# castacks/mvs_gi

Measured on AMD Instinct MI355X. Metric: stereo frames/sec/GPU (G16V, 3-cam, D=16) + inv-dist L1 vs reference, higher is better.
Workload: dtype f16x3 (split-fp16 MFMA operands: 11 + 11 significant bits, f32 accumulate/activations)

## Files before the change

### mvs_gi_amd/csrc/conv3d.hip

```cpp
#include "common.hpp"
#include "conv_common.hpp"
#include "conv3d_variants.hpp"
#ifdef MVSGI_STAMPS
#include <cstdio>
#include <cstdlib>
#endif

namespace {

__global__ void pack_head_weights_kernel(const float* __restrict__ w, float* __restrict__ wp, int Cin) {
    const int idx = blockIdx.x * 256 + threadIdx.x;
    if (idx >= 27 * Cin) return;
    const int tap = idx / Cin, ci = idx % Cin;
    wp[idx] = w[ci * 27 + tap];
}

#include "conv3d_f32mfma.hpp"
#include "conv3d_bf16x3.hpp"


__global__ __launch_bounds__(256) void conv3d_head_kernel(ConvArgs a, int dchunk, int nd) {
    constexpr int TH = 8, TW = 32, ITH = TH + 2, ITW = TW + 2, PV = ITH * ITW;
    constexpr int NT = (PV + 31) / 32;
    constexpr int TPW = (NT + 3) / 4;
// ... 199 lines not shown
    MVSGI_REQUIRE((long long)a.Hin * a.Win * a.Cin < (1ll << 31), "conv3d(head): plane too large for 32-bit offsets");
    hipLaunchKernelGGL(conv3d_head_kernel, dim3((unsigned)nt), dim3(256), lds_bytes, st, a, dchunk, (int)nd);
    return mvsgi::check_launch("mvsgi_conv3d_f32(head)");
}

int launch_direct(const ConvArgs& a, hipStream_t st) {
    const long long vox = (long long)a.B * a.Do * a.Ho * a.Wo;
    if (a.Cout == 1) {
        hipLaunchKernelGGL((conv3d_direct_kernel<1>), dim3((unsigned)mvsgi::cdiv(vox, 256)), dim3(256), 0, st, a);
    } else {
        const long long total = vox * mvsgi::cdiv(a.Cout, 4);
        hipLaunchKernelGGL((conv3d_direct_kernel<4>), dim3((unsigned)mvsgi::cdiv(total, 256)), dim3(256), 0, st, a);
    }
    return mvsgi::check_launch("mvsgi_conv3d_f32(direct)");
}

bool v32_applies(const ConvArgs& a) {
    if (a.Cout % 32 || a.Cin % 16 || a.stride != 1) return false;
    const long long big = (long long)a.B * mvsgi::cdiv(a.Do, 4) * mvsgi::cdiv(a.Ho, 4) * mvsgi::cdiv(a.Wo, 16);
    const long long mid = (long long)a.B * mvsgi::cdiv(a.Do, 2) * mvsgi::cdiv(a.Ho, 4) * mvsgi::cdiv(a.Wo, 16);
    return a.Cout == 32 ? big >= 384 : mid * mvsgi::cdiv(a.Cout, 64) >= 384;
}

int select_variant_up2(const ConvArgs& a, int w_layout) {
    if (w_layout == MVSGI_CONV_BF16X3_D32) {
        const int base = a.Cin % 32 ? V_COUNT : select_variant_up2(a, MVSGI_CONV_BF16X3);
        const bool d2 = a.Do == 2;
        if (base == B3U_N64) return d2 ? B3DU2_N64 : B3DU_N64;
        if (base == B3U_N96) return d2 ? B3DU2_N96 : B3DU_N96;
        mvsgi::fail("mvsgi_conv3d_up2_f32: the 32-channel-slice kernels do not apply to this problem (see mvsgi_conv3d_up2_d32_applies)");
        return V_COUNT;
    }
    const bool c16_layout = w_layout == MVSGI_CONV_BF16X3_C16;
    if (w_layout == MVSGI_CONV_BF16X3_V32) {
        if (!v32_applies(a) || !a.wp) { mvsgi::fail("mvsgi_conv3d_up2_f32: the 32x32x16 kernel does not apply to this problem"); return V_COUNT; }
        return a.Cout == 32 ? B3VU_N32 : B3VU_N64;
    }
    if (a.Cin % 16 || a.Cout % 16) {
        mvsgi::fail("mvsgi_conv3d_up2_f32: Cin, Cout must be multiples of 16 (got %d, %d)", a.Cin, a.Cout);
        return V_COUNT;
    }
    if (!a.wp) { mvsgi::fail("mvsgi_conv3d_up2_f32: needs w_packed (bf16x3 layout)"); return V_COUNT; }
    const int CT = a.Cout / 16;
    const long long big = (long long)a.B * mvsgi::cdiv(a.Do, 4) * mvsgi::cdiv(a.Ho, 4) * mvsgi::cdiv(a.Wo, 16);
    const long long mid = (long long)a.B * mvsgi::cdiv(a.Do, 2) * mvsgi::cdiv(a.Ho, 4) * mvsgi::cdiv(a.Wo, 16);
    if (CT == 1) return c16_layout ? B3PU_N16 : B3U_N16;
    if (CT == 2) {
        if (big >= 384) return B3U_N32;
        const long long cus = mvsgi::device_cus(), r32 = mvsgi::cdiv(big, cus), rm = mvsgi::cdiv(mid, cus);
        return 157 * (100 + 85 * (r32 - 1)) < 100 * (100 + 85 * (rm - 1)) ? B3U_N32 : B3U_N32_M;
    }
    if (CT == 3) return B3U_N48;
    if (CT % 6 == 0 && mid * (CT / 6) >= 384) return B3U_N96;
    if (CT % 2 == 0 && (long long)a.B * mvsgi::cdiv(a.Do, 2) * mvsgi::cdiv(a.Ho, 2) * mvsgi::cdiv(a.Wo, 16) * (CT / 2) <= mvsgi::device_cus())
        return B3U_N32_TB;
    return B3U_N64;
}

int select_variant(const ConvArgs& a, int impl);

int d32_variant(const ConvArgs& a) {
    if (a.stride != 1 || a.Cin % 32 || a.Cout % 16) return V_COUNT;
    ConvArgs b = a;
    static const float dummy = 0.f;
    if (!b.wp) b.wp = reinterpret_cast<const f32x4*>(&dummy);
    const bool d2 = a.Do == 2;
    switch (select_variant(b, MVSGI_CONV_BF16X3)) {
        case B3_N64: return d2 ? B3D2_N64 : B3D_N64;
        case B3_N64_H5: return d2 ? B3D2_N64_H5 : B3D_N64_H5;
        case B3_N64_W8: return d2 ? B3D2_N64_W8 : B3D_N64_W8;
        case B3_N96: return d2 ? B3D2_N96 : B3D_N96;
        case B3_N96_H5: return d2 ? B3D2_N96_H5 : B3D_N96_H5;
        case B3_N96_W8: return d2 ? B3D2_N96_W8 : B3D_N96_W8;
        case B3_N128_P: return B3D_N128_P;
        case B3_N128_PH5: return B3D_N128_PH5;
        case B3_N128_PW8: return B3D_N128_PW8;
        case B3_N192_PH5: return B3D_N192_PH5;
        case B3_N192_PW8: return B3D_N192_PW8;
        case B3_N16_TW: return d2 && a.Cout % 32 == 0 ? B3D2_N32_TB : V_COUNT;
        case B3_N32_TB: return d2 ? B3D2_N32_TB : B3D_N32_TB;
        case B3_N64_S: return d2 ? B3D2_N64_S : B3D_N64_S;
        default: return V_COUNT;
    }
}

// ... 398 lines not shown
```

### mvs_gi_amd/csrc/conv3d_bf16x3.hpp

```cpp
#pragma once
#ifndef MVSGI_ABL
#define MVSGI_ABL 0
#endif

#include "split_fmt.hpp"

constexpr int kVSB = 80;

__device__ __forceinline__ void split_bf16x4(const f32x4 x, u32x2& hi, u32x2& lo) {
#pragma unroll
    for (int p = 0; p < 2; ++p) {
        const f32x2 v = {x[2 * p], x[2 * p + 1]};
        const unsigned hb = __builtin_bit_cast(unsigned, __builtin_convertvector(v, bf16x2));
        const f32x2 hf = {__builtin_bit_cast(float, hb << 16), __builtin_bit_cast(float, hb & 0xffff0000u)};
        hi[p] = hb;
        float r0 = v[0] - hf[0], r1 = v[1] - hf[1];
        asm volatile("" : "+v"(r0));
        asm volatile("" : "+v"(r1));
        lo[p] = __builtin_bit_cast(unsigned, __builtin_convertvector(f32x2{r0, r1}, bf16x2));
    }
}
__device__ __forceinline__ f32x4 fma4(const f32x4 a, const f32x4 b, const f32x4 c) {
    f32x4 r;
#pragma unroll
// ... 142 lines not shown
    if (idx >= total) return;
    const int lane = (int)(idx & 63);
    long long r = idx >> 6;
    const int tap = (int)(r % 27);
    r /= 27;
    const int ct = (int)(r % CT);
    const int cc = (int)(r / CT);
    const int co = ct * 32 + (lane & 31);
    const int ci = cc * 16 + (lane >> 5) * 8;
    u16x8 hi, lo;
    for (int j = 0; j < 8; ++j) {
        const float v = w[((long long)co * Cin + ci + j) * 27 + tap];
        unsigned short h_, l_;
        split_weight(v, f16, h_, l_);
        hi[j] = h_;
        lo[j] = l_;
    }
    const long long o = ((((long long)cc * CT + ct) * 27 + tap) * 2) * 64 + lane;
    wp[o] = __builtin_bit_cast(bf16x8, hi);
    wp[o + 64] = __builtin_bit_cast(bf16x8, lo);
}

template <int NW, int MW, int WM, int WN, int TD, int TH, int TW, int S, int KD, bool UPS, bool PLANE, bool V32, bool WLDS, bool F16, bool D32 = false, int DK = 3, int BRD = 0>
__device__ __forceinline__ void conv3d_x3_body(const ConvArgs& a) {
    static_assert(!WLDS || (WN == 1 && KD == 3 && !UPS && !PLANE && !V32 && S == 1 && NW == 1 && MW <= 2), "LDS-staged weights: one shared cout tile, one or two voxel tiles per wave");
    static_assert(!V32 || (S == 1 && KD == 3 && TW == 16 && TH % 2 == 0 && !PLANE), "32x32x16 schedule: stride 1, 16-wide even bricks");
    static_assert(!PLANE || (NW == 1 && WN == 1 && WM == 4 && TH == 4 && MW == TD && TW == 16 && S == 1 && KD == 3),
                  "plane schedule: Cout == 16, 4 h-rows x TD planes x 16 w per brick");
    static_assert(!UPS || (S == 1 && KD == 3 && TD % 2 == 0 && TH % 2 == 0 && TW % 2 == 0),
                  "fused upsample: stride 1, even bricks (halo bricks are whole 2x2x2 cells)");
    static_assert(WM * WN == 4, "4 consumer waves per workgroup");
    static_assert(WM * MW * (V32 ? 32 : 16) == TD * TH * TW, "brick must be covered by the voxel tiles");
    static_assert(KD == 3 || (KD == 1 && TD == 1), "2-D bricks are one plane thick");
    constexpr int SD = KD == 1 ? 1 : S;
    static_assert(!D32 || (KD == 3 && S == 1 && !PLANE && !V32 && !WLDS), "32-channel slices: stride-1 3x3x3 variants (plain or fused upsample) only");
    static_assert(DK == 3 || (D32 && DK >= 1 && (TD == 1 ? DK <= 2 : (TD == 2 && WM == 2 && MW * 16 == TH * TW))), "depth skip: one- or two-plane bricks whose waves own whole planes");
    constexpr bool DKU = D32 && TD == 1 && DK == 2;
    constexpr int kTaps = KD * 9, kPairs = D32 ? 9 * DK : pairs_of(KD);
    constexpr int kWBlk = D32 ? 27 : kPairs;
    constexpr int ITD = (TD - 1) * SD + KD, ITH = (TH - 1) * S + 3, ITW = (TW - 1) * S + 3;
    constexpr int IV = ITD * ITH * ITW;
    constexpr int QB = D32 ? 3 : 2;
    constexpr int NIT = (IV * (1 << QB) + 255) / 256;
    constexpr int ROWP = V32 ? ((ITW * kVSB + 255) / 256) * 256 : ITW * kVSB;
    constexpr int SUB = ITD * ITH * ROWP;
    constexpr int BUF = D32 ? 2 * SUB : SUB;
    constexpr int WB = WLDS ? (MW * NW == 1 ? 8 : 4) :
// ... 2 lines not shown
                       NW <= 2 ? 4 : 2;
    constexpr int LA = WB - 1;
    constexpr int NSLOT = ((kPairs + WB - 1) / WB) * WB;
    static_assert(NSLOT % WB == 0 && NSLOT >= kPairs, "pipeline geometry");
    constexpr bool RPRE = MW * NW <= 8;
#ifndef MVSGI_WARM
#define MVSGI_WARM 0
#endif
    constexpr bool WARM = MVSGI_WARM && KD == 3 && !UPS && !PLANE && !V32 && !WLDS && S == 1 && MW * NW <= 2;

    constexpr int WBYTES = WLDS ? NW * kPairs * 2048 : 0;
    constexpr int BUFW = BUF + WBYTES;
    constexpr int WARM_LDS = 2 * BUFW;
    extern __shared__ __attribute__((aligned(16))) unsigned char ldsb[];
    float satm = 0.f;

    const int tid = threadIdx.x, lane = tid & 63;
    const int wave = __builtin_amdgcn_readfirstlane(tid >> 6);
    const bool producer = wave >= 4;
    const int CT = a.Cout / (V32 ? 32 : 16);
    const int ny = (CT + WN * NW - 1) / (WN * NW);
    const int nchunks = a.Cin / (D32 ? 32 : 16);
    const int total = a.total_units;
    const int G = gridDim.x;
    const int nmine = (total - (int)blockIdx.x + G - 1) / G;
    const int U = nmine * nchunks;
#ifdef MVSGI_STAMPS
    int nst = 0;
#define STAMP()                                                                                     \
    if (a.dbg && blockIdx.x == 8 && nst < 120) {                                                    \
        unsigned long long t_;                                                                      \
        asm volatile("s_memtime %0\n\ts_waitcnt lgkmcnt(0)" : "=s"(t_)::"memory");                  \
        if (lane == 0) a.dbg[wave * 128 + nst] = t_;                                                \
        nst++;                                                                                      \
    }
#else
#define STAMP()
#endif
    STAMP()

#define MVSGI_DECODE_DH(T, OD, OH, B) { OD = (T % a.tiles_d) * TD + a.od_off; T /= a.tiles_d; OH = (T % a.tiles_h) * TH; B = T / a.tiles_h; }
#define MVSGI_DECODE(ID, CB, B, OD, OH, OW)                       \
    {                                                             \
        int t_ = xcd_remap((ID), total);                          \
        CB = t_ % ny;                                             \
        t_ /= ny;                                                 \
        OW = (t_ % a.tiles_w) * TW;                               \
        t_ /= a.tiles_w;                                          \
// ... 18 lines not shown
            f32x4 crA[NITU][8], crB[NITU][8];
            unsigned imA[NITU], imB[NITU];
#define MVSGI_PLAN_UPS(UNIT)                                                                            \
            {                                                                                           \
                int cb_, b_, od_, oh_, ow_;                                                             \
                MVSGI_DECODE(UNIT, cb_, b_, od_, oh_, ow_)                                              \
                (void)cb_;                                                                              \
                _Pragma("unroll") for (int it = 0; it < NITU; ++it) {                                   \
                    const int c = MVSGI_UPS_CQ(it) >> QB;                                               \
                    const int cw = c % CW, ch = (c / CW) % CH, cd = c / (CW * CH);                      \
                    const int gd = od_ - 1 + 2 * cd, gh = oh_ - 1 + 2 * ch, gw = ow_ - 1 + 2 * cw;      \
                    lo_d[it] = (gd - 1) >> 1;                                                           \
                    lo_h[it] = (gh - 1) >> 1;                                                           \
                    lo_w[it] = (gw - 1) >> 1;                                                           \
                    inmask[it] = (gd >= 0 && gd < a.Din ? 1u : 0u) | (gd + 1 < a.Din ? 2u : 0u) |       \
                                 (gh >= 0 && gh < a.Hin ? 4u : 0u) | (gh + 1 < a.Hin ? 8u : 0u) |       \
                                 (gw >= 0 && gw < a.Win ? 16u : 0u) | (gw + 1 < a.Win ? 32u : 0u);      \
                }                                                                                       \
                xb = a.x + (long long)b_ * Dl * Hl * Wl * a.Cin;                                        \
            }
#define MVSGI_CLAMP(V, N) ((V) < 0 ? 0 : ((V) > (N) - 1 ? (N) - 1 : (V)))
            int k2 = 0, cc2 = 0;
#define MVSGI_ISSUE_UPS_BEGIN()                                                                         \
            if (cc2 == 0 && k2 > 0) { MVSGI_PLAN_UPS((int)blockIdx.x + k2 * G) }
#define MVSGI_ISSUE_UPS1(CR, IM, IT)                                                                    \
            {                                                                                           \
                const int q = MVSGI_UPS_CQ(IT) & ((1 << QB) - 1);                                       \
                const bool live = MVSGI_UPS_LIVE(IT);                                                   \
                const int d0 = live ? MVSGI_CLAMP(lo_d[IT], Dl) : 0, d1 = live ? MVSGI_CLAMP(lo_d[IT] + 1, Dl) : 0; \
                const int h0 = live ? MVSGI_CLAMP(lo_h[IT], Hl) : 0, h1 = live ? MVSGI_CLAMP(lo_h[IT] + 1, Hl) : 0; \
                const int w0 = live ? MVSGI_CLAMP(lo_w[IT], Wl) : 0, w1 = live ? MVSGI_CLAMP(lo_w[IT] + 1, Wl) : 0; \
                const int cofs = cc2 * (D32 ? 32 : 16) + q * 4;                                         \
                 \
                const int od_[2] = {__mul24(d0, sD_), __mul24(d1, sD_)}, oh_[2] = {__mul24(h0, sH_), __mul24(h1, sH_)};   \
                const int ow_[2] = {__mul24(w0, a.Cin) + cofs, __mul24(w1, a.Cin) + cofs};              \
                _Pragma("unroll") for (int k = 0; k < 8; ++k)                                           \
                    CR[IT][k] = *reinterpret_cast<const f32x4*>(xb + (od_[(k >> 2) & 1] + oh_[(k >> 1) & 1] + ow_[k & 1])); \
                IM[IT] = inmask[IT];                                                                    \
            }
#define MVSGI_ISSUE_UPS_END()                                                                           \
            {                                                                                           \
                if (++cc2 == nchunks) { cc2 = 0; ++k2; }                                                \
                if (k2 >= nmine) { k2 = nmine - 1; cc2 = nchunks - 1; }                                 \
            }
#define MVSGI_ISSUE_UPS(CR, IM)                                                                         \
            {                                                                                           \
                MVSGI_ISSUE_UPS_BEGIN()                                                                 \
// ... 56 lines not shown
                                const bool ok = ((IM[IT] >> kd) & (IM[IT] >> (2 + kh)) & (IM[IT] >> (4 + kw)) & 1u) != 0; \
                                u32x2 hi, lo;                                                           \
                                split_x4<F16>(xo[kd][kh][kw], hi, lo, satm);                                   \
                                if (!ok) hi = lo = u32x2{0u, 0u};                                       \
                                const int vo_ = ((2 * cd + kd) * ITH + 2 * ch + kh) * ROWP + (2 * cw + kw) * kVSB; \
                                *reinterpret_cast<u32x2*>((DST) + sub_ + vo_ + q * 8) = hi;             \
                                *reinterpret_cast<u32x2*>((DST) + sub_ + vo_ + 32 + q * 8) = lo;        \
                            }                                                                           \
                }                                                                                       \
            }
#define MVSGI_PUT_UPS(CR, IM, DST)                                                                      \
            { _Pragma("unroll") for (int it = 0; it < NITU; ++it) MVSGI_PUT_UPS1(CR, IM, DST, it) }
#define MVSGI_STEP_UPS(NEW, IMNEW, OLD, IMOLD, DST, DOPUT)                                              \
            {                                                                                           \
                MVSGI_ISSUE_UPS_BEGIN()                                                                 \
                _Pragma("unroll") for (int it = 0; it < NITU; ++it) {                                   \
                    MVSGI_ISSUE_UPS1(NEW, IMNEW, it)                                                    \
                    if (DOPUT) MVSGI_PUT_UPS1(OLD, IMOLD, DST, it)                                      \
                    __builtin_amdgcn_sched_barrier(0);                                                  \
                }                                                                                       \
                MVSGI_ISSUE_UPS_END()                                                                   \
            }
            STAMP()
            MVSGI_PLAN_UPS((int)blockIdx.x)
            MVSGI_ISSUE_UPS(crA, imA)
            MVSGI_PUT_UPS(crA, imA, ldsb)
            MVSGI_ISSUE_UPS(crA, imA)
            STAMP()
            __syncthreads();
            STAMP()
            for (int u = 0; u < U; u += 2) {
                MVSGI_STEP_UPS(crB, imB, crA, imA, ldsb + ((u + 1) & 1) * BUF, u + 1 < U)
                STAMP()
                __syncthreads();
                STAMP()
                if (u + 1 < U) {
                    MVSGI_STEP_UPS(crA, imA, crB, imB, ldsb + ((u + 2) & 1) * BUF, u + 2 < U)
                    STAMP()
                    __syncthreads();
                    STAMP()
                }
            }
#undef MVSGI_ISSUE_UPS
#undef MVSGI_PUT_UPS
#undef MVSGI_LERP2
#undef MVSGI_ISSUE_UPS_BEGIN
#undef MVSGI_ISSUE_UPS1
// ... 36 lines not shown
#define MVSGI_PLAN(UNIT)                                                                                \
        {                                                                                               \
            int cb_, b_, od_, oh_, ow_;                                                                 \
            MVSGI_DECODE(UNIT, cb_, b_, od_, oh_, ow_)                                                  \
            pct0 = cb_ * NW < CT - NW ? cb_ * NW : CT - NW;                                             \
            wct0 = cb_ * (WN * NW) < CT - WN * NW ? cb_ * (WN * NW) : (CT > WN * NW ? CT - WN * NW : 0);   \
            const int id0_ = od_ * SD - KD / 2, ih0_ = oh_ * S - 1, iw0_ = ow_ * S - 1;                 \
            const int bbase_ = ((id0_ * a.Hin + ih0_) * a.Win + iw0_) * a.Cin * 4;                      \
            _Pragma("unroll") for (int it = 0; it < NIT; ++it) {                                        \
                const unsigned gd = (unsigned)(id0_ + (int)(cpk[it] & 255u));                           \
                const unsigned gh = (unsigned)(ih0_ + (int)((cpk[it] >> 8) & 255u));                    \
                const unsigned gw = (unsigned)(iw0_ + (int)(cpk[it] >> 16));                            \
                const bool ok = gd < (unsigned)a.Din && gh < (unsigned)a.Hin && gw < (unsigned)a.Win;   \
                                                  \
                 \
                goff[it] = !ok ? (int)0x80000000 : D32 ? (((int)gd * a.Hin + (int)gh) * a.Win + (int)gw) * a.Cin * 4 + ((ptid + it * 256) & 7) * 16 \
                                                       : ibase[it] + bbase_;                           \
            }                                                                                           \
            xdesc = __builtin_amdgcn_make_buffer_rsrc(const_cast<float*>(a.x) + (long long)b_ * a.Din * a.Hin * a.Win * a.Cin, 0, \
                                                      a.Din * a.Hin * a.Win * a.Cin * 4, kRawBufferFlags);  \
        }
        int k2 = 0, cc2 = 0;
#define MVSGI_ISSUE_BEGIN()                                                                             \
        if (cc2 == 0 && k2 > 0) { MVSGI_PLAN((int)blockIdx.x + k2 * G) }
#define MVSGI_ISSUE1(PRE, IT)                                                                           \
        PRE[IT] = __builtin_bit_cast(f32x4, __builtin_amdgcn_raw_buffer_load_b128(xdesc, goff[IT] + cc2 * (D32 ? 128 : 64), 0, 0));
#define MVSGI_ISSUE_END(OK)                                                                             \
        {                                                                                               \
            if (++cc2 == nchunks) { cc2 = 0; ++k2; }                                                    \
            if (k2 >= nmine) { k2 = nmine - 1; cc2 = nchunks - 1; }    \
        }
#define MVSGI_WISSUE(WPRE)       \
        if constexpr (WLDS) {                                                                           \
            const char* ws_ = wsrc + ((long long)cc2 * CT + pct0) * (kPairs * 2048);                     \
            _Pragma("unroll") for (int it = 0; it < WNIT; ++it) WPRE[it] = *reinterpret_cast<const f32x4*>(ws_ + it * 4096); \
        }
#define MVSGI_WARM_ISSUE()       \
        if constexpr (WARM) {                                                                           \
            const unsigned wo_ = (unsigned)(((long long)cc2 * CT + wct0) * (kPairs * 2048)) + (unsigned)((wave - 4) * 1024 + lane * 16); \
            _Pragma("unroll") for (int it = 0; it < WN * NW * kPairs * 2048 / 4096; ++it)               \
                LDS_DMA16(wdesc, ldsb + WARM_LDS + (wave - 4) * 1024, wo_ + it * 4096u, 0, 0);          \
        }
#define MVSGI_WPUT(WPRE, DST)                                                                           \
        if constexpr (WLDS) {                                                                           \
            _Pragma("unroll") for (int it = 0; it < WNIT; ++it)                                         \
                *reinterpret_cast<f32x4*>((DST) + BUF + (wave - 4) * 1024 + lane * 16 + it * 4096) = WPRE[it]; \
        }
// ... 19 lines not shown
                }                                                                                       \
                const int vo_ = V32 ? (v / ITW) * ROWP + (v % ITW) * kVSB : v * kVSB;                   \
                *reinterpret_cast<u32x2*>((DST) + sub_ + vo_ + q * 8) = hi;                             \
                *reinterpret_cast<u32x2*>((DST) + sub_ + vo_ + 32 + q * 8) = lo;                        \
            }                                                                                           \
        }
#define MVSGI_PUT(PRE, OK, DST)                                                                         \
        { _Pragma("unroll") for (int it = 0; it < NIT; ++it) if (!MVSGI_ITEM_DEAD(it)) MVSGI_PUT1(PRE, OK, DST, it) }
#define MVSGI_STEP(NEW, OKNEW, OLD, OKOLD, DST, DOPUT, WNEW, WOLD)                                      \
        {                                                                                               \
            MVSGI_ISSUE_BEGIN()                                                                         \
            MVSGI_WARM_ISSUE()                                                                          \
            MVSGI_WISSUE(WNEW)                                                                          \
            if (DOPUT) { MVSGI_WPUT(WOLD, DST) }                                                        \
            _Pragma("unroll") for (int it = 0; it < NIT; ++it) {                                        \
                if (MVSGI_ITEM_DEAD(it)) continue;                                                      \
                MVSGI_ISSUE1(NEW, it)                                                                   \
                if (DOPUT) MVSGI_PUT1(OLD, OKOLD, DST, it)                                              \
                __builtin_amdgcn_sched_barrier(0);                                                      \
            }                                                                                           \
            MVSGI_ISSUE_END(OKNEW)                                                                      \
        }
        STAMP()
        MVSGI_PLAN((int)blockIdx.x)
        MVSGI_ISSUE(preA, okA, wpreA)
        MVSGI_PUT(preA, okA, ldsb)
        MVSGI_WPUT(wpreA, ldsb)
        MVSGI_ISSUE(preA, okA, wpreA)
        STAMP()
        __syncthreads();
        STAMP()
        for (int u = 0; u < U; u += 2) {
            MVSGI_STEP(preB, okB, preA, okA, ldsb + ((u + 1) & 1) * BUFW, u + 1 < U && !(MVSGI_ABL & 8), wpreB, wpreA)
            STAMP()
            __syncthreads();
            STAMP()
            if (u + 1 < U) {
                MVSGI_STEP(preA, okA, preB, okB, ldsb + ((u + 2) & 1) * BUFW, u + 2 < U && !(MVSGI_ABL & 8), wpreA, wpreB)
                STAMP()
                __syncthreads();
                STAMP()
            }
        }
#undef MVSGI_ISSUE
#undef MVSGI_WISSUE
#undef MVSGI_WPUT
#undef MVSGI_WARM_ISSUE
// ... 37 lines not shown
            for (int j = 0; j < NW; ++j)
#pragma unroll
                for (int e = 0; e < 16; ++e) acc[i][j][e] = 0.f;
#define MVSGI_V_LOADW(BUFI, CC, T, CTS)                                                                \
        _Pragma("unroll") for (int j = 0; j < NW; ++j) {                                               \
            const char* q_ = wpb + (((long long)(CC) * CT + CTS[j]) * 27 + (T)) * 2048;   \
            wh[BUFI][j] = *reinterpret_cast<const bf16x8*>(q_ + l16);                                  \
            wl[BUFI][j] = *reinterpret_cast<const bf16x8*>(q_ + l16 + 1024u);                          \
        }
#define MVSGI_V_READX(BUFI, T)                                                                         \
        {                                                                                              \
            const int off_ = (((T) / 9) * ITH + ((T) / 3) % 3) * ROWP + ((T) % 3) * kVSB;              \
            _Pragma("unroll") for (int i = 0; i < MW; ++i) {                                           \
                xh[BUFI][i] = *reinterpret_cast<const bf16x8*>(img + xbase[i] + off_);                 \
                xl[BUFI][i] = *reinterpret_cast<const bf16x8*>(img + xbase[i] + off_ + 32);            \
            }                                                                                          \
        }
#define MVSGI_V_MFMAS(WBUFI, BUFI)                                                                          \
        _Pragma("unroll") for (int tr = 0; tr < 3; ++tr)                                               \
            _Pragma("unroll") for (int i = 0; i < MW; ++i)                                             \
                _Pragma("unroll") for (int j = 0; j < NW; ++j)                                         \
                    acc[i][j] = mfma32<F16>(tr == 0 ? wl[WBUFI][j] : wh[WBUFI][j], tr == 1 ? xl[BUFI][i] : xh[BUFI][i], acc[i][j]);
        int cb_, b_, od0, oh0, ow0;
        MVSGI_DECODE((int)blockIdx.x, cb_, b_, od0, oh0, ow0)
        MVSGI_CTILES(ctc, cb_)
        {
            unsigned l16 = lane16;
#pragma unroll
            for (int t0 = 0; t0 < LAW; ++t0) { MVSGI_V_LOADW(t0, 0, t0, ctc) }
        }
        STAMP()
        __syncthreads();
        STAMP()
        int k = 0, cc = 0;
        for (int u = 0; u < U; ++u) {
            const unsigned char* img = ldsb + (u & 1) * BUF;
            const bool last = cc + 1 == nchunks;
            const bool more = u + 1 < U;
            const int ncc = last ? 0 : cc + 1;
            int ncb = cb_, nb = b_, nod0 = od0, noh0 = oh0, now0 = ow0;
            if (last && more) {
                MVSGI_DECODE((int)blockIdx.x + (k + 1) * G, ncb, nb, nod0, noh0, now0)
                MVSGI_CTILES(ctn, ncb)
            } else {
#pragma unroll
                for (int j = 0; j < NW; ++j) ctn[j] = ctc[j];
            }
            int eoff[MW];
            f32x4 rres[MW][NW][4], esc[NW][4], esh[NW][4];
            if (last) {
#pragma unroll
                for (int j = 0; j < NW; ++j)
#pragma unroll
                    for (int g = 0; g < 4; ++g) {
                        esc[j][g] = *reinterpret_cast<const f32x4*>(a.scale + ctc[j] * 32 + 8 * g + 4 * kh2);
                        esh[j][g] = *reinterpret_cast<const f32x4*>(a.shift + ctc[j] * 32 + 8 * g + 4 * kh2);
                    }
#pragma unroll
                for (int i = 0; i < MW; ++i) {
                    const int od = od0 + tdv[i], oh = oh0 + thv[i], ow = ow0 + twv[i];
                    const bool inside = od < a.Do && oh < a.Ho && ow < a.Wo;
                    eoff[i] = inside ? ((od * a.Ho + oh) * a.Wo + ow) * a.Cout + kh2 * 4 : -1;
                }
            }
            MVSGI_V_READX(0, 0)
// ... 135 lines not shown
            }                                                                                         \
        }
#define MVSGI_MFMAS(WBUF, XBUF, I0, I1)                                                               \
        _Pragma("unroll") for (int i = (I0); i < (I1); ++i)                                           \
            _Pragma("unroll") for (int j = 0; j < NW; ++j)                                            \
                acc[i][j] = mfma16<F16>(wl[WBUF][j], xh[XBUF][i], acc[i][j]); \
        _Pragma("unroll") for (int i = (I0); i < (I1); ++i)                                           \
            _Pragma("unroll") for (int j = 0; j < NW; ++j)                                            \
                (TACC ? acc1[i][j] : acc[i][j]) = mfma16<F16>(wh[WBUF][j], xl[XBUF][i], TACC ? acc1[i][j] : acc[i][j]); \
        _Pragma("unroll") for (int i = (I0); i < (I1); ++i)                                           \
            _Pragma("unroll") for (int j = 0; j < NW; ++j)                                            \
                (TACC ? acc2[i][j] : acc[i][j]) = mfma16<F16>(wh[WBUF][j], xh[XBUF][i], TACC ? acc2[i][j] : acc[i][j]);
        constexpr bool TACC = KD == 3 && !PLANE && !V32 && MW * NW <= 2;
        f32x4 acc[MW][NW], acc1[MW][NW], acc2[MW][NW];
#pragma unroll
        for (int i = 0; i < MW; ++i)
#pragma unroll
            for (int j = 0; j < NW; ++j) {
                acc[i][j] = f32x4{0.f, 0.f, 0.f, 0.f};
                if (TACC) acc1[i][j] = acc2[i][j] = f32x4{0.f, 0.f, 0.f, 0.f};
            }

        int cb_, b_, od0, oh0, ow0;
        MVSGI_DECODE((int)blockIdx.x, cb_, b_, od0, oh0, ow0)
        MVSGI_CTILES(ctc, cb_)
        constexpr int NPP = 5;
        constexpr int PD = PLANE ? TD + 2 : 1;
        bf16x8 pwh[3][PLANE ? 3 : 1], pwl[3][PLANE ? 3 : 1];
        bf16x8 pxh[2][PD], pxl[2][PD];
        const int pbase = (wm * ITW + col) * kVSB + (kg >> 1) * 16;
#define MVSGI_PL_LOADW(BUFI, CC, P)                                                                    \
        _Pragma("unroll") for (int kd = 0; kd < 3; ++kd) {                                             \
            const char* q_ = wpb + ((long long)(((CC) * NPP + (P)) * 3 + kd)) * 2048;    \
            pwh[BUFI][kd] = *reinterpret_cast<const bf16x8*>(q_ + l16);                                \
            pwl[BUFI][kd] = *reinterpret_cast<const bf16x8*>(q_ + l16 + 1024u);                        \
        }
#define MVSGI_PL_READX(BUFI, P)                                                                        \
        {                                                                                              \
            const int t0_ = 2 * (P), t1_ = 2 * (P) + 1 < 9 ? 2 * (P) + 1 : 2 * (P);                    \
            const int o0_ = ((t0_ / 3) * ITW + t0_ % 3) * kVSB, o1_ = ((t1_ / 3) * ITW + t1_ % 3) * kVSB; \
            const int off_ = pbase + (second ? o1_ : o0_);                                             \
            _Pragma("unroll") for (int ip = 0; ip < PD; ++ip) {                                        \
                pxh[BUFI][ip] = *reinterpret_cast<const bf16x8*>(img + off_ + ip * (ITH * ITW * kVSB)); \
                pxl[BUFI][ip] = *reinterpret_cast<const bf16x8*>(img + off_ + ip * (ITH * ITW * kVSB) + 32); \
            }                                                                                          \
        }
#define MVSGI_PL_MFMAS(WBUFI, BUFI)                                                                         \
// ... 1 lines not shown
            _Pragma("unroll") for (int kd = 0; kd < 3; ++kd)                                           \
                _Pragma("unroll") for (int i = 0; i < TD; ++i)                                         \
                    acc[i][0] = mfma16<F16>(tr == 0 ? pwl[WBUFI][kd] : pwh[WBUFI][kd], tr == 1 ? pxl[BUFI][i + kd] : pxh[BUFI][i + kd], acc[i][0]);
        if constexpr (PLANE) {
            unsigned l16 = lane16;
            MVSGI_PL_LOADW(0, 0, 0)
            MVSGI_PL_LOADW(1, 0, 1)
        } else if constexpr (!WLDS) {
            unsigned l16 = lane16;
#pragma unroll
            for (int s0 = 0; s0 < LA; ++s0) { MVSGI_LOADWB(wpb + (DKU && od0 == 0 ? 9 * 2048 : 0), s0, 0, s0, ctc) }
        }
        STAMP()
        __syncthreads();
        STAMP()
        int k = 0, cc = 0;
        for (int u = 0; u < U; ++u) {
            const unsigned char* img = ldsb + (u & 1) * BUFW + (DKU && od0 == 0 ? ITH * ITW * kVSB : 0);
            const bool last = cc + 1 == nchunks;
            const bool more = u + 1 < U;
            const int ncc = last ? 0 : cc + 1;
            int ncb = cb_, nb = b_, nod0 = od0, noh0 = oh0, now0 = ow0;
            if (last && more) {
                MVSGI_DECODE((int)blockIdx.x + (k + 1) * G, ncb, nb, nod0, noh0, now0)
                MVSGI_CTILES(ctn, ncb)
            } else {
#pragma unroll
                for (int j = 0; j < NW; ++j) ctn[j] = ctc[j];
            }
            const char* const wpc_ = wpb + (DKU && od0 == 0 ? 9 * 2048 : 0);
            const char* const wpn_ = wpb + (DKU && nod0 == 0 ? 9 * 2048 : 0);
            f32x4 esc[NW], esh[NW], rres[RPRE ? MW : 1][RPRE ? NW : 1];
            int eoff[MW];
            int soff[MW];
            const int ypd = a.ys_2d ? 0 : 1, ypp = a.ys_2d ? 2 : 1;
#pragma unroll
            for (int j = 0; j < NW; ++j) {
                esc[j] = *reinterpret_cast<const f32x4*>(a.scale + ctc[j] * 16 + kg * 4);
                esh[j] = *reinterpret_cast<const f32x4*>(a.shift + ctc[j] * 16 + kg * 4);
            }
            if (last) {
#pragma unroll
                for (int i = 0; i < MW; ++i) {
                    const int od = od0 + tdv[i], oh = oh0 + thv[i], ow = ow0 + twv[i];
                    const bool inside = od < a.Do && oh < a.Ho && ow < a.Wo;
                    eoff[i] = inside ? ((od * a.Ho + oh) * a.Wo + ow) * a.Cout + kg * 4 : -1;
                    soff[i] = ((((od + ypd) * (a.Ho + 2 * ypp) + oh + ypp) * (a.Wo + 2 * ypp) + ow + ypp) * a.Cout) * 4 + (kg >> 1) * 16 + (kg & 1) * 8;
// ... 133 lines not shown
                for (int j = 0; j < NW; ++j) ctc[j] = ctn[j];
            }
            cc = ncc;
            STAMP()
            __syncthreads();
            STAMP()
        }
#undef MVSGI_T0
#undef MVSGI_T1
#undef MVSGI_TAP
#undef MVSGI_PL_LOADW
#undef MVSGI_PL_READX
#undef MVSGI_PL_MFMAS
#undef MVSGI_CTILES
#undef MVSGI_LOADW
#undef MVSGI_READX
#undef MVSGI_MFMAS
    }
#undef MVSGI_DECODE
    STAMP()
#undef STAMP
    if constexpr (F16) sf_sat_report(a.sat, kSatSplit, satm, 65504.f);
}

template <int NW, int MW, int WM, int WN, int TD, int TH, int TW, int S, int KD = 3, bool UPS = false, bool PLANE = false,
          bool V32 = false, bool WLDS = false>
__global__ __launch_bounds__(512, 2) void conv3d_bf16x3_kernel(ConvArgs a) {
    conv3d_x3_body<NW, MW, WM, WN, TD, TH, TW, S, KD, UPS, PLANE, V32, WLDS, false>(a);
}
template <int NW, int MW, int WM, int WN, int TD, int TH, int TW, int S, int KD = 3, bool UPS = false, bool PLANE = false,
          bool V32 = false, bool WLDS = false>
__global__ __launch_bounds__(512, 2) void conv3d_f16x3_kernel(ConvArgs a) {
    conv3d_x3_body<NW, MW, WM, WN, TD, TH, TW, S, KD, UPS, PLANE, V32, WLDS, true>(a);
}

template <int NW, int MW, int WM, int WN, int TD, int TH, int TW>
__global__ __launch_bounds__(512, 2) void conv3d_bf16x3_d32_kernel(ConvArgs a) {
    conv3d_x3_body<NW, MW, WM, WN, TD, TH, TW, 1, 3, false, false, false, false, false, true>(a);
}
template <int NW, int MW, int WM, int WN, int TD, int TH, int TW>
__global__ __launch_bounds__(512, 2) void conv3d_f16x3_d32_kernel(ConvArgs a) {
    conv3d_x3_body<NW, MW, WM, WN, TD, TH, TW, 1, 3, false, false, false, false, true, true>(a);
}

template <int NW, int MW, int WM, int WN, int TD, int TH, int TW>
__global__ __launch_bounds__(512, 2) void conv3d_bf16x3_d32_dk_kernel(ConvArgs a) {
// ... 16 lines not shown
__global__ __launch_bounds__(512, 2) void conv3d_bf16x3_d32_dk2_kernel(ConvArgs a) {
    conv3d_x3_body<NW, MW, WM, WN, TD, TH, TW, 1, 3, false, false, false, false, false, true, 2>(a);
}
template <int NW, int MW, int WM, int WN, int TD, int TH, int TW>
__global__ __launch_bounds__(512, 2) void conv3d_f16x3_d32_dk2_kernel(ConvArgs a) {
    conv3d_x3_body<NW, MW, WM, WN, TD, TH, TW, 1, 3, false, false, false, false, true, true, 2>(a);
}

template <int NW, int MW, int WM, int WN, int TD, int TH, int TW, int BRD>
__global__ __launch_bounds__(512, 2) void conv3d_bf16x3_d32_brd_kernel(ConvArgs a) {
    conv3d_x3_body<NW, MW, WM, WN, TD, TH, TW, 1, 3, false, false, false, false, false, true, 3, BRD>(a);
}
template <int NW, int MW, int WM, int WN, int TD, int TH, int TW, int BRD>
__global__ __launch_bounds__(512, 2) void conv3d_f16x3_d32_brd_kernel(ConvArgs a) {
    conv3d_x3_body<NW, MW, WM, WN, TD, TH, TW, 1, 3, false, false, false, false, true, true, 3, BRD>(a);
}
template <int NW, int MW, int WM, int WN, int TD, int TH, int TW, int BRD>
__global__ __launch_bounds__(512, 2) void conv3d_bf16x3_d32u_brd_kernel(ConvArgs a) {
    conv3d_x3_body<NW, MW, WM, WN, TD, TH, TW, 1, 3, true, false, false, false, false, true, 3, BRD>(a);
}
template <int NW, int MW, int WM, int WN, int TD, int TH, int TW, int BRD>
__global__ __launch_bounds__(512, 2) void conv3d_f16x3_d32u_brd_kernel(ConvArgs a) {
    conv3d_x3_body<NW, MW, WM, WN, TD, TH, TW, 1, 3, true, false, false, false, true, true, 3, BRD>(a);
}

template <int NW, int MW, int WM, int WN, int TD, int TH, int TW>
__global__ __launch_bounds__(512, 2) void conv3d_bf16x3_d32u_kernel(ConvArgs a) {
    conv3d_x3_body<NW, MW, WM, WN, TD, TH, TW, 1, 3, true, false, false, false, false, true>(a);
}
template <int NW, int MW, int WM, int WN, int TD, int TH, int TW>
__global__ __launch_bounds__(512, 2) void conv3d_f16x3_d32u_kernel(ConvArgs a) {
    conv3d_x3_body<NW, MW, WM, WN, TD, TH, TW, 1, 3, true, false, false, false, true, true>(a);
}

template <int NW, int MW, int WM, int WN, int TD, int TH, int TW, int S, int KD = 3, bool UPS = false, bool PLANE = false,
          bool V32 = false, bool WLDS = false, bool F16 = false, bool D32 = false, bool DSK = false, int BRD = 0>
int launch_bf16x3(ConvArgs a, hipStream_t st) {
    constexpr int ITD = (TD - 1) * (KD == 1 ? 1 : S) + KD, ITH = (TH - 1) * S + 3, ITW = (TW - 1) * S + 3;
    constexpr int ROWP = V32 ? ((ITW * kVSB + 255) / 256) * 256 : ITW * kVSB;
    constexpr bool WARM = MVSGI_WARM && KD == 3 && !UPS && !PLANE && !V32 && !WLDS && S == 1 && MW * NW <= 2;
    static_assert(!D32 || (S == 1 && KD == 3 && !PLANE && !V32 && !WLDS), "32-channel slices: stride-1 3x3x3 variants");
    constexpr size_t lds_bytes = (size_t)2 * ((D32 ? 2 : 1) * ITD * ITH * ROWP + (WLDS ? NW * pairs_of(KD) * 2048 : 0)) + (WARM ? 4096 : 0);
    static_assert(lds_bytes <= 160 * 1024, "LDS images too large");
    void (*kern)(ConvArgs);
    static_assert(!DSK || (D32 && TD <= 2), "depth skip: 32-channel slices, one- or two-plane bricks");
    constexpr bool DKU = DSK && BRD == 3;
    static_assert(!DKU || (TD == 1 && !UPS), "per-unit depth skip: one-plane bricks");
    MVSGI_REQUIRE(!DSK || a.Do == (DKU ? 2 : TD), "conv3d: the depth-skip kernels serve volumes exactly %d planes deep (got %d)", DKU ? 2 : TD, a.Do);
    if constexpr (DKU && F16) kern = conv3d_f16x3_d32_dk2_kernel<NW, MW, WM, WN, TD, TH, TW>;
    else if constexpr (DKU) kern = conv3d_bf16x3_d32_dk2_kernel<NW, MW, WM, WN, TD, TH, TW>;
    else if constexpr (BRD != 0 && UPS && F16) kern = conv3d_f16x3_d32u_brd_kernel<NW, MW, WM, WN, TD, TH, TW, BRD>;
    else if constexpr (BRD != 0 && UPS) kern = conv3d_bf16x3_d32u_brd_kernel<NW, MW, WM, WN, TD, TH, TW, BRD>;
    else if constexpr (BRD != 0 && F16) kern = conv3d_f16x3_d32_brd_kernel<NW, MW, WM, WN, TD, TH, TW, BRD>;
    else if constexpr (BRD != 0) kern = conv3d_bf16x3_d32_brd_kernel<NW, MW, WM, WN, TD, TH, TW, BRD>;
    else if constexpr (DSK && UPS && F16) kern = conv3d_f16x3_d32u_dk_kernel<NW, MW, WM, WN, TD, TH, TW>;
    else if constexpr (DSK && UPS) kern = conv3d_bf16x3_d32u_dk_kernel<NW, MW, WM, WN, TD, TH, TW>;
    else if constexpr (DSK && F16) kern = conv3d_f16x3_d32_dk_kernel<NW, MW, WM, WN, TD, TH, TW>;
    else if constexpr (DSK) kern = conv3d_bf16x3_d32_dk_kernel<NW, MW, WM, WN, TD, TH, TW>;
    else if constexpr (D32 && UPS && F16) kern = conv3d_f16x3_d32u_kernel<NW, MW, WM, WN, TD, TH, TW>;
    else if constexpr (D32 && UPS) kern = conv3d_bf16x3_d32u_kernel<NW, MW, WM, WN, TD, TH, TW>;
    else if constexpr (D32 && F16) kern = conv3d_f16x3_d32_kernel<NW, MW, WM, WN, TD, TH, TW>;
    else if constexpr (D32) kern = conv3d_bf16x3_d32_kernel<NW, MW, WM, WN, TD, TH, TW>;
    else if constexpr (F16) kern = conv3d_f16x3_kernel<NW, MW, WM, WN, TD, TH, TW, S, KD, UPS, PLANE, V32, WLDS>;
    else kern = conv3d_bf16x3_kernel<NW, MW, WM, WN, TD, TH, TW, S, KD, UPS, PLANE, V32, WLDS>;
    MVSGI_REQUIRE(!D32 || a.Cin % 32 == 0, "conv3d: the 32-channel-slice kernels need Cin %% 32 == 0 (got %d)", a.Cin);
    static mvsgi::PersistentGeom geo_cache[mvsgi::kMaxDevices] = {};
    mvsgi::PersistentGeom geo;
    if (mvsgi::persistent_geometry(kern, 512, lds_bytes, 2, geo_cache, "conv3d(bf16x3)", geo)) return 1;
    a.tiles_h = (int)mvsgi::cdiv(a.Ho, TH);
    a.tiles_w = (int)mvsgi::cdiv(a.Wo, TW);
    const int CT = a.Cout / (V32 ? 32 : 16);
    constexpr bool kBorderSplit = D32 && !DSK && BRD == 0 && TD == 2 && WM == 2 && MW == 4 && TH == 4 && TW == 16 && S == 1;
    if constexpr (kBorderSplit) {
        const long long layer = (long long)a.B * a.tiles_h * a.tiles_w * mvsgi::cdiv(CT, WN * NW);
        if (a.od_cnt == 0 && a.Do == 4 && layer >= 4ll * geo.cus) {
            ConvArgs b = a;
            b.od_cnt = 1;
            b.od_off = 0;
            if (launch_bf16x3<NW, MW, WM, WN, TD, TH, TW, S, KD, UPS, PLANE, V32, WLDS, F16, D32, DSK, 1>(b, st)) return 1;
            b.od_off = 2;
            return launch_bf16x3<NW, MW, WM, WN, TD, TH, TW, S, KD, UPS, PLANE, V32, WLDS, F16, D32, DSK, 2>(b, st);
        }
    }
    a.tiles_d = a.od_cnt > 0 ? a.od_cnt : (int)mvsgi::cdiv(a.Do, TD);
    const long long nb = (long long)a.B * a.tiles_d * a.tiles_h * a.tiles_w * mvsgi::cdiv(CT, WN * NW);
    MVSGI_REQUIRE(nb < (1ll << 31), "conv3d: too many units");
    MVSGI_REQUIRE((long long)a.Din * a.Hin * a.Win * a.Cin < (1ll << 29), "conv3d: volume too large for 32-bit byte offsets");
    MVSGI_REQUIRE(!UPS || (a.Din % 2 == 0 && a.Hin % 2 == 0 && a.Win % 2 == 0), "conv3d: fused upsample needs even sizes");
    MVSGI_REQUIRE(!UPS || (long long)(a.Hin / 2) * (a.Win / 2) * a.Cin < (1ll << 23), "conv3d: fused upsample: low-resolution plane too large for 24-bit strides");
    MVSGI_REQUIRE((long long)a.Do * a.Ho * a.Wo * a.Cout < (1ll << 31), "conv3d: output frame too large for 32-bit element offsets");
    MVSGI_REQUIRE(!a.y_split || (!V32 && (long long)(a.Do + 2) * (a.Ho + 4) * (a.Wo + 4) * a.Cout * 4 < (1ll << 31)),
                  "conv3d: split-padded output not available for this kernel / size");
    a.total_units = (int)nb;
    MVSGI_SAT_WORDS(sat_words_);
    a.sat = sat_words_;
#ifdef MVSGI_STAMPS
    {
        static unsigned long long* dbgbuf = nullptr;
        const char* e_ = getenv("MVSGI_STAMP");
        if (e_ && !dbgbuf) { (void)hipMalloc(&dbgbuf, 8 * 128 * 8); (void)hipMemset(dbgbuf, 0, 8 * 128 * 8); }
        a.dbg = dbgbuf;
        if (e_ && atoi(e_) == 2 && dbgbuf) {
            static unsigned long long h[8 * 128];
            (void)hipDeviceSynchronize();
            (void)hipMemcpy(h, dbgbuf, sizeof(h), hipMemcpyDeviceToHost);
            for (int w = 0; w < 8; ++w) {
                fprintf(stderr, "wave %d:", w);
                for (int i = 0; i < 120; ++i) fprintf(stderr, " %lld", (long long)(h[w * 128 + i] - h[0]));
                fprintf(stderr, "\n");
            }
        }
    }
#endif
    const long long resident = ((long long)geo.cus * geo.wgs_per_cu) / 8 * 8 > 0 ? ((long long)geo.cus * geo.wgs_per_cu) / 8 * 8 : 8;
    const unsigned grid = (unsigned)(nb <= resident ? nb : resident);
    hipLaunchKernelGGL(kern, dim3(grid), dim3(512), lds_bytes, st, a);
    return mvsgi::check_launch("mvsgi_conv3d_f32(bf16x3)");
}
```

Before: 6629.

## Merge the two depth-border conv launches into one persistent launch

Adds a BRD=4 kernel that runs both depth-border halves (od_off 0 and TD) in a single launch. Workgroups are split into interleaved groups of eight, each with its own rank and stride, and the conv body now takes an explicit block index and grid size. The default environment mode (1) uses this single launch in place of two back-to-back launches, which is meant to remove a kernel launch and the tail idle time between them. The trade-off is fewer workgroups per half when the resident limit caps the doubled grid, plus mode 2, which forces the border split and the 64/96-wide variants.

After: 6634 (median of 5 runs). No clear change (+0.1%).

```diff
diff --git a/mvs_gi_amd/csrc/conv3d.hip b/mvs_gi_amd/csrc/conv3d.hip
--- a/mvs_gi_amd/csrc/conv3d.hip
+++ b/mvs_gi_amd/csrc/conv3d.hip
@@ -245,8 +245,14 @@
     return a.Cout == 32 ? big >= 384 : mid * mvsgi::cdiv(a.Cout, 64) >= 384;
 }
 
+int brd_test_variant(const ConvArgs& a, int n64, int n96) {
+    if (!(brd_launch_mode() & 2) || a.stride != 1 || a.Do != 4 || a.Cin % 32) return V_COUNT;
+    return a.Cout % 96 == 0 ? n96 : a.Cout % 64 == 0 ? n64 : V_COUNT;
+}
+
 int select_variant_up2(const ConvArgs& a, int w_layout) {
     if (w_layout == MVSGI_CONV_BF16X3_D32) {
+        if (const int v = brd_test_variant(a, B3DU_N64, B3DU_N96); v != V_COUNT) return v;
         const int base = a.Cin % 32 ? V_COUNT : select_variant_up2(a, MVSGI_CONV_BF16X3);
         const bool d2 = a.Do == 2;
         if (base == B3U_N64) return d2 ? B3DU2_N64 : B3DU_N64;
@@ -284,6 +290,7 @@
 
 int d32_variant(const ConvArgs& a) {
     if (a.stride != 1 || a.Cin % 32 || a.Cout % 16) return V_COUNT;
+    if (const int v = brd_test_variant(a, B3D_N64, B3D_N96); v != V_COUNT) return v;
     ConvArgs b = a;
     static const float dummy = 0.f;
     if (!b.wp) b.wp = reinterpret_cast<const f32x4*>(&dummy);
diff --git a/mvs_gi_amd/csrc/conv3d_bf16x3.hpp b/mvs_gi_amd/csrc/conv3d_bf16x3.hpp
--- a/mvs_gi_amd/csrc/conv3d_bf16x3.hpp
+++ b/mvs_gi_amd/csrc/conv3d_bf16x3.hpp
@@ -188,7 +188,7 @@
 }
 
 template <int NW, int MW, int WM, int WN, int TD, int TH, int TW, int S, int KD, bool UPS, bool PLANE, bool V32, bool WLDS, bool F16, bool D32 = false, int DK = 3, int BRD = 0>
-__device__ __forceinline__ void conv3d_x3_body(const ConvArgs& a) {
+__device__ __forceinline__ void conv3d_x3_body(const ConvArgs& a, const int BLK, const int G) {
     static_assert(!WLDS || (WN == 1 && KD == 3 && !UPS && !PLANE && !V32 && S == 1 && NW == 1 && MW <= 2), "LDS-staged weights: one shared cout tile, one or two voxel tiles per wave");
     static_assert(!V32 || (S == 1 && KD == 3 && TW == 16 && TH % 2 == 0 && !PLANE), "32x32x16 schedule: stride 1, 16-wide even bricks");
     static_assert(!PLANE || (NW == 1 && WN == 1 && WM == 4 && TH == 4 && MW == TD && TW == 16 && S == 1 && KD == 3),
@@ -237,8 +237,7 @@
     const int ny = (CT + WN * NW - 1) / (WN * NW);
     const int nchunks = a.Cin / (D32 ? 32 : 16);
     const int total = a.total_units;
-    const int G = gridDim.x;
-    const int nmine = (total - (int)blockIdx.x + G - 1) / G;
+    const int nmine = (total - BLK + G - 1) / G;
     const int U = nmine * nchunks;
 #ifdef MVSGI_STAMPS
     int nst = 0;
@@ -303,7 +302,7 @@
 #define MVSGI_CLAMP(V, N) ((V) < 0 ? 0 : ((V) > (N) - 1 ? (N) - 1 : (V)))
             int k2 = 0, cc2 = 0;
 #define MVSGI_ISSUE_UPS_BEGIN()                                                                         \
-            if (cc2 == 0 && k2 > 0) { MVSGI_PLAN_UPS((int)blockIdx.x + k2 * G) }
+            if (cc2 == 0 && k2 > 0) { MVSGI_PLAN_UPS(BLK + k2 * G) }
 #define MVSGI_ISSUE_UPS1(CR, IM, IT)                                                                    \
             {                                                                                           \
                 const int q = MVSGI_UPS_CQ(IT) & ((1 << QB) - 1);                                       \
@@ -406,7 +405,7 @@
                 MVSGI_ISSUE_UPS_END()                                                                   \
             }
             STAMP()
-            MVSGI_PLAN_UPS((int)blockIdx.x)
+            MVSGI_PLAN_UPS(BLK)
             MVSGI_ISSUE_UPS(crA, imA)
             MVSGI_PUT_UPS(crA, imA, ldsb)
             MVSGI_ISSUE_UPS(crA, imA)
@@ -489,7 +488,7 @@
         }
         int k2 = 0, cc2 = 0;
 #define MVSGI_ISSUE_BEGIN()                                                                             \
-        if (cc2 == 0 && k2 > 0) { MVSGI_PLAN((int)blockIdx.x + k2 * G) }
+        if (cc2 == 0 && k2 > 0) { MVSGI_PLAN(BLK + k2 * G) }
 #define MVSGI_ISSUE1(PRE, IT)                                                                           \
         PRE[IT] = __builtin_bit_cast(f32x4, __builtin_amdgcn_raw_buffer_load_b128(xdesc, goff[IT] + cc2 * (D32 ? 128 : 64), 0, 0));
 #define MVSGI_ISSUE_END(OK)                                                                             \
@@ -555,7 +554,7 @@
             MVSGI_ISSUE_END(OKNEW)                                                                      \
         }
         STAMP()
-        MVSGI_PLAN((int)blockIdx.x)
+        MVSGI_PLAN(BLK)
         MVSGI_ISSUE(preA, okA, wpreA)
         MVSGI_PUT(preA, okA, ldsb)
         MVSGI_WPUT(wpreA, ldsb)
@@ -639,7 +638,7 @@
                 _Pragma("unroll") for (int j = 0; j < NW; ++j)                                         \
                     acc[i][j] = mfma32<F16>(tr == 0 ? wl[WBUFI][j] : wh[WBUFI][j], tr == 1 ? xl[BUFI][i] : xh[BUFI][i], acc[i][j]);
         int cb_, b_, od0, oh0, ow0;
-        MVSGI_DECODE((int)blockIdx.x, cb_, b_, od0, oh0, ow0)
+        MVSGI_DECODE(BLK, cb_, b_, od0, oh0, ow0)
         MVSGI_CTILES(ctc, cb_)
         {
             unsigned l16 = lane16;
@@ -657,7 +656,7 @@
             const int ncc = last ? 0 : cc + 1;
             int ncb = cb_, nb = b_, nod0 = od0, noh0 = oh0, now0 = ow0;
             if (last && more) {
-                MVSGI_DECODE((int)blockIdx.x + (k + 1) * G, ncb, nb, nod0, noh0, now0)
+                MVSGI_DECODE(BLK + (k + 1) * G, ncb, nb, nod0, noh0, now0)
                 MVSGI_CTILES(ctn, ncb)
             } else {
 #pragma unroll
@@ -839,7 +838,7 @@
             }
 
         int cb_, b_, od0, oh0, ow0;
-        MVSGI_DECODE((int)blockIdx.x, cb_, b_, od0, oh0, ow0)
+        MVSGI_DECODE(BLK, cb_, b_, od0, oh0, ow0)
         MVSGI_CTILES(ctc, cb_)
         constexpr int NPP = 5;
         constexpr int PD = PLANE ? TD + 2 : 1;
@@ -887,7 +886,7 @@
             const int ncc = last ? 0 : cc + 1;
             int ncb = cb_, nb = b_, nod0 = od0, noh0 = oh0, now0 = ow0;
             if (last && more) {
-                MVSGI_DECODE((int)blockIdx.x + (k + 1) * G, ncb, nb, nod0, noh0, now0)
+                MVSGI_DECODE(BLK + (k + 1) * G, ncb, nb, nod0, noh0, now0)
                 MVSGI_CTILES(ctn, ncb)
             } else {
 #pragma unroll
@@ -1067,6 +1066,10 @@
 #undef STAMP
     if constexpr (F16) sf_sat_report(a.sat, kSatSplit, satm, 65504.f);
 }
+template <int NW, int MW, int WM, int WN, int TD, int TH, int TW, int S, int KD, bool UPS, bool PLANE, bool V32, bool WLDS, bool F16, bool D32 = false, int DK = 3, int BRD = 0>
+__device__ __forceinline__ void conv3d_x3_body(const ConvArgs& a) {
+    conv3d_x3_body<NW, MW, WM, WN, TD, TH, TW, S, KD, UPS, PLANE, V32, WLDS, F16, D32, DK, BRD>(a, (int)blockIdx.x, (int)gridDim.x);
+}
 
 template <int NW, int MW, int WM, int WN, int TD, int TH, int TW, int S, int KD = 3, bool UPS = false, bool PLANE = false,
           bool V32 = false, bool WLDS = false>
@@ -1129,6 +1132,46 @@
 template <int NW, int MW, int WM, int WN, int TD, int TH, int TW, int BRD>
 __global__ __launch_bounds__(512, 2) void conv3d_f16x3_d32u_brd_kernel(ConvArgs a) {
     conv3d_x3_body<NW, MW, WM, WN, TD, TH, TW, 1, 3, true, false, false, false, true, true, 3, BRD>(a);
+}
+
+template <int NW, int MW, int WM, int WN, int TD, int TH, int TW, bool UPS, bool F16>
+__device__ __forceinline__ void conv3d_x3_brd2_body(const ConvArgs& a) {
+    const int id = blockIdx.x, grid = gridDim.x;
+    const bool top = (id >> 3) & 1;
+    const int rank = ((id >> 4) << 3) | (id & 7);
+    const int sixteen = (grid >> 4) << 3, rest = grid & 15;
+    const int mates = sixteen + (top ? (rest > 8 ? rest - 8 : 0) : (rest < 8 ? rest : 8));
+    const int G = mates < a.total_units ? mates : a.total_units;
+    if (rank >= G) return;
+    ConvArgs b = a;
+    if (!top) {
+        b.od_off = 0;
+        conv3d_x3_body<NW, MW, WM, WN, TD, TH, TW, 1, 3, UPS, false, false, false, F16, true, 3, 1>(b, rank, G);
+    } else {
+        b.od_off = TD;
+        conv3d_x3_body<NW, MW, WM, WN, TD, TH, TW, 1, 3, UPS, false, false, false, F16, true, 3, 2>(b, rank, G);
+    }
+}
+template <int NW, int MW, int WM, int WN, int TD, int TH, int TW>
+__global__ __launch_bounds__(512, 2) void conv3d_bf16x3_d32_brd2_kernel(ConvArgs a) {
+    conv3d_x3_brd2_body<NW, MW, WM, WN, TD, TH, TW, false, false>(a);
+}
+template <int NW, int MW, int WM, int WN, int TD, int TH, int TW>
+__global__ __launch_bounds__(512, 2) void conv3d_f16x3_d32_brd2_kernel(ConvArgs a) {
+    conv3d_x3_brd2_body<NW, MW, WM, WN, TD, TH, TW, false, true>(a);
+}
+template <int NW, int MW, int WM, int WN, int TD, int TH, int TW>
+__global__ __launch_bounds__(512, 2) void conv3d_bf16x3_d32u_brd2_kernel(ConvArgs a) {
+    conv3d_x3_brd2_body<NW, MW, WM, WN, TD, TH, TW, true, false>(a);
+}
+template <int NW, int MW, int WM, int WN, int TD, int TH, int TW>
+__global__ __launch_bounds__(512, 2) void conv3d_f16x3_d32u_brd2_kernel(ConvArgs a) {
+    conv3d_x3_brd2_body<NW, MW, WM, WN, TD, TH, TW, true, true>(a);
+}
+
+inline int brd_launch_mode() {
+    const char* e = getenv("MVSGI_BRD_ONE_LAUNCH");
+    return e && *e ? atoi(e) & 3 : 1;
 }
 
 template <int NW, int MW, int WM, int WN, int TD, int TH, int TW>
@@ -1156,6 +1199,10 @@
     MVSGI_REQUIRE(!DSK || a.Do == (DKU ? 2 : TD), "conv3d: the depth-skip kernels serve volumes exactly %d planes deep (got %d)", DKU ? 2 : TD, a.Do);
     if constexpr (DKU && F16) kern = conv3d_f16x3_d32_dk2_kernel<NW, MW, WM, WN, TD, TH, TW>;
     else if constexpr (DKU) kern = conv3d_bf16x3_d32_dk2_kernel<NW, MW, WM, WN, TD, TH, TW>;
+    else if constexpr (BRD == 4 && UPS && F16) kern = conv3d_f16x3_d32u_brd2_kernel<NW, MW, WM, WN, TD, TH, TW>;
+    else if constexpr (BRD == 4 && UPS) kern = conv3d_bf16x3_d32u_brd2_kernel<NW, MW, WM, WN, TD, TH, TW>;
+    else if constexpr (BRD == 4 && F16) kern = conv3d_f16x3_d32_brd2_kernel<NW, MW, WM, WN, TD, TH, TW>;
+    else if constexpr (BRD == 4) kern = conv3d_bf16x3_d32_brd2_kernel<NW, MW, WM, WN, TD, TH, TW>;
     else if constexpr (BRD != 0 && UPS && F16) kern = conv3d_f16x3_d32u_brd_kernel<NW, MW, WM, WN, TD, TH, TW, BRD>;
     else if constexpr (BRD != 0 && UPS) kern = conv3d_bf16x3_d32u_brd_kernel<NW, MW, WM, WN, TD, TH, TW, BRD>;
     else if constexpr (BRD != 0 && F16) kern = conv3d_f16x3_d32_brd_kernel<NW, MW, WM, WN, TD, TH, TW, BRD>;
@@ -1180,10 +1227,12 @@
     constexpr bool kBorderSplit = D32 && !DSK && BRD == 0 && TD == 2 && WM == 2 && MW == 4 && TH == 4 && TW == 16 && S == 1;
     if constexpr (kBorderSplit) {
         const long long layer = (long long)a.B * a.tiles_h * a.tiles_w * mvsgi::cdiv(CT, WN * NW);
-        if (a.od_cnt == 0 && a.Do == 4 && layer >= 4ll * geo.cus) {
+        const int mode = brd_launch_mode();
+        if (a.od_cnt == 0 && a.Do == 4 && (layer >= 4ll * geo.cus || (mode & 2))) {
             ConvArgs b = a;
             b.od_cnt = 1;
             b.od_off = 0;
+            if (mode & 1) return launch_bf16x3<NW, MW, WM, WN, TD, TH, TW, S, KD, UPS, PLANE, V32, WLDS, F16, D32, DSK, 4>(b, st);
             if (launch_bf16x3<NW, MW, WM, WN, TD, TH, TW, S, KD, UPS, PLANE, V32, WLDS, F16, D32, DSK, 1>(b, st)) return 1;
             b.od_off = 2;
             return launch_bf16x3<NW, MW, WM, WN, TD, TH, TW, S, KD, UPS, PLANE, V32, WLDS, F16, D32, DSK, 2>(b, st);
@@ -1220,7 +1269,11 @@
     }
 #endif
     const long long resident = ((long long)geo.cus * geo.wgs_per_cu) / 8 * 8 > 0 ? ((long long)geo.cus * geo.wgs_per_cu) / 8 * 8 : 8;
-    const unsigned grid = (unsigned)(nb <= resident ? nb : resident);
+    unsigned grid = (unsigned)(nb <= resident ? nb : resident);
+    if constexpr (BRD == 4) {
+        const long long both = 2 * ((nb + 7) / 8 * 8), room = resident >= 16 ? resident : 16;
+        grid = (unsigned)(both <= room ? both : room);
+    }
     hipLaunchKernelGGL(kern, dim3(grid), dim3(512), lds_bytes, st, a);
     return mvsgi::check_launch("mvsgi_conv3d_f32(bf16x3)");
 }
```
